# LouisBearing/BirdSoundClassif

Hardware: AMD Instinct MI355X
Metric: clips/sec (3 s @ 22.05 kHz) detect fwd (higher is better)
Workload: dtype f32; 1 GPU; BASELINE.json configs[1]: 1xMI355X inference, batch=64 synthetic 3 s clips (PCM16 @22.05 kHz resident in HBM) through the HIP STFT front end + detector forward + device post-processing, detections returned to the host; batch_per_gpu=64, distinct_clips=64, lanes=2

## Files before the change

### birdsoundclassif_amd/_lib.py

```python
import ctypes as C
import os
import subprocess

_HERE = os.path.dirname(os.path.abspath(__file__))
LIB_PATH = os.environ.get('NBM_LIB') or os.path.join(_HERE, 'libnbm_hip.so')
CSRC = os.path.join(_HERE, 'csrc')

_lib = None


class GemmDesc(C.Structure):
    _fields_ = [('x', C.c_void_p), ('w', C.c_void_p), ('y', C.c_void_p),
                ('scale', C.c_void_p), ('shift', C.c_void_p), ('residual', C.c_void_p),
                ('x_gs', C.c_int64), ('w_gs', C.c_int64), ('y_gs', C.c_int64), ('res_gs', C.c_int64),
                ('groups', C.c_int),
                ('B', C.c_int), ('H', C.c_int), ('W', C.c_int), ('Cin', C.c_int),
                ('N', C.c_int),
                ('kh', C.c_int), ('kw', C.c_int), ('stride', C.c_int), ('pad', C.c_int),
                ('Ho', C.c_int), ('Wo', C.c_int),
                ('x_ld', C.c_int), ('w_ld', C.c_int), ('y_ld', C.c_int), ('res_ld', C.c_int),
                ('alpha', C.c_float), ('act', C.c_int), ('shift_per_row', C.c_int),
                ('up', C.c_void_p), ('up_H', C.c_int), ('up_W', C.c_int),
                ('rows', C.c_void_p), ('rows_blocks', C.c_void_p),
                ('rows_mode', C.c_int), ('rows_count', C.c_int), ('rows_TH', C.c_int), ('rows_TW', C.c_int),
                ('mask', C.c_void_p), ('mask_ld', C.c_int), ('bits_out', C.c_void_p)]


class GconvDesc(C.Structure):
    _fields_ = [('x', C.c_void_p), ('w', C.c_void_p), ('y', C.c_void_p), ('scale', C.c_void_p), ('shift', C.c_void_p),
                ('B', C.c_int), ('H', C.c_int), ('W', C.c_int), ('groups', C.c_int), ('Cg', C.c_int),
                ('kh', C.c_int), ('kw', C.c_int), ('stride', C.c_int), ('pad', C.c_int), ('Ho', C.c_int), ('Wo', C.c_int),
                ('x_ld', C.c_int), ('y_ld', C.c_int), ('relu', C.c_int)]


class GconvBwdDesc(C.Structure):
    _fields_ = [('g', C.c_void_p), ('y', C.c_void_p), ('w', C.c_void_p), ('x', C.c_void_p), ('out', C.c_void_p),
                ('scale', C.c_void_p), ('workspace', C.c_void_p), ('workspace_bytes', C.c_longlong),
                ('B', C.c_int), ('H', C.c_int), ('W', C.c_int), ('groups', C.c_int), ('Cg', C.c_int),
                ('kh', C.c_int), ('kw', C.c_int), ('stride', C.c_int), ('pad', C.c_int), ('Ho', C.c_int), ('Wo', C.c_int),
                ('g_ld', C.c_int), ('y_ld', C.c_int), ('x_ld', C.c_int), ('out_ld', C.c_int),
                ('accumulate', C.c_int), ('splits', C.c_int)]


class RoiDesc(C.Structure):
    _fields_ = [('fmap', C.c_void_p * 5), ('fh', C.c_int * 5), ('fw', C.c_int * 5),
                ('n_levels', C.c_int), ('C', C.c_int),
                ('rois', C.c_void_p), ('n_roi', C.c_void_p), ('B', C.c_int), ('roi_cap', C.c_int),
                ('pe_f', C.c_void_p), ('pe_t', C.c_void_p), ('img_h', C.c_int), ('img_w', C.c_int),
                ('pool', C.c_void_p), ('pe', C.c_void_p), ('level', C.c_void_p)]


class AugmentParams(C.Structure):
    _fields_ = [('gain', C.c_float), ('coef', C.c_float), ('denom', C.c_float), ('neg_coef', C.c_float),
                ('neg_denom', C.c_float), ('flags', C.c_int32), ('hard_index', C.c_int32), ('pad', C.c_int32),
                ('noise_seed', C.c_uint64)]


class BwdDesc(C.Structure):
    _fields_ = [('g', C.c_void_p), ('w', C.c_void_p), ('x', C.c_void_p), ('out', C.c_void_p),
                ('a_scale', C.c_void_p), ('row_scale', C.c_void_p), ('residual', C.c_void_p), ('mask', C.c_void_p),
                ('g_gs', C.c_int64), ('w_gs', C.c_int64), ('x_gs', C.c_int64), ('out_gs', C.c_int64), ('res_gs', C.c_int64),
                ('groups', C.c_int),
                ('B', C.c_int), ('H', C.c_int), ('W', C.c_int), ('Cin', C.c_int), ('N', C.c_int),
                ('kh', C.c_int), ('kw', C.c_int), ('stride', C.c_int), ('pad', C.c_int), ('Ho', C.c_int), ('Wo', C.c_int),
                ('g_ld', C.c_int), ('w_ld', C.c_int), ('x_ld', C.c_int), ('out_ld', C.c_int), ('res_ld', C.c_int),
                ('mask_ld', C.c_int), ('alpha', C.c_float), ('bias_grad', C.c_void_p), ('residual2', C.c_void_p), ('res2_ld', C.c_int),
                ('mask_bits', C.c_void_p)]


class GemmPlan(C.Structure):
    _fields_ = [('name', C.c_char_p), ('rc', C.c_int), ('kernel', C.c_int), ('grid', C.c_int * 3), ('block', C.c_int),
                ('m_tiles', C.c_int), ('n_tiles', C.c_int), ('vec_epi', C.c_int), ('fast', C.c_int), ('slices', C.c_int),
                ('phased', C.c_int), ('ph_tiles', C.c_int * 4), ('splits', C.c_int), ('k_chunk', C.c_int),
                ('plain', C.c_int), ('b_generic', C.c_int), ('narrow_m', C.c_int), ('halves', C.c_int)]


_P, _I, _L, _F, _U64 = C.c_void_p, C.c_int, C.c_int64, C.c_float, C.c_uint64

SIGNATURES = {
    'nbm_graph_census': [_P, C.POINTER(C.c_longlong * 6)],
    'nbm_copy_rect': [_P, _P, _L, _L, _I, _L, _L, _I, _I, _P],
    'nbm_gemm_conv': [C.POINTER(GemmDesc), _P],
    'nbm_gconv3x3': [C.POINTER(GconvDesc), _P],
    'nbm_gconv3x3_dgrad': [C.POINTER(GconvBwdDesc), _P],
    'nbm_gconv3x3_wgrad': [C.POINTER(GconvBwdDesc), _P],
    'nbm_gconv3x3_wgrad_workspace': [C.POINTER(GconvBwdDesc), C.POINTER(C.c_longlong)],
    'nbm_pcm16_to_wave': [_P, _L, _I, _I, _I, _P, _L, _L, _P, _L, _I, _I, _P],
    'nbm_resample_to_wave': [_P, _L, _I, _L, _I, _I, _P, _I, _L, _L, _P, _L, _I, _I, _I, _P],
    'nbm_wav_decode': [_P, _L, _I, _I, _I, _I, _L, _P, _L, _P],
    'nbm_minmax_init': [_P, _I, _P],
    'nbm_stft_db': [_P, _L, _I, _I, _I, _I, _P, _I, _I, _I, _F, _P, _L, _I, _P, _P],
    'nbm_spec_windows': [_P, _L, _I, _I, _I, _I, _P, _P, _I, _I, _I, _P, _P],
    'nbm_spec_windows_table': [_P, _I, _I, _P, _I, _I, _P],
    'nbm_init_conv': [_P, _L, _P, _P, _I, _P, _P],
    'nbm_stem7x7': [_P, _I, _I, _I, _P, _P, _P, _P, _P, _P, _P],
    'nbm_stem7x7_wgrad': [_P, _P, _I, _I, _I, _P, _P, _P],
    'nbm_maxpool3x3s2': [_P, _I, _I, _I, _I, _P, _I, _I, _P, _P],
    'nbm_space_to_batch2': [_P, _I, _I, _I, _I, _P, _I, _P],
    'nbm_avgpool2x2': [_P, _I, _I, _I, _I, _P, _P],
    'nbm_avgpool2x2_bwd': [_P, _I, _I, _I, _I, _P, _P],
    'nbm_upsample_bilinear_add': [_P, _I, _I, _I, _I, _P, _P, _I, _I, _P],
    'nbm_softmax_rows': [_P, _L, _I, _L, _P],
    'nbm_dwconv3x3': [_P, _I, _I, _I, _I, _I, _I, _P, _P, _P, _L, _P, _I, _I, _P],
    'nbm_silu': [_P, _P, _L, _P],
    'nbm_layernorm': [_P, _L, _I, _P, _P, _F, _P, _P],
    'nbm_mha_small': [_P, _P, _P, _I, _I, _I, _P, _I, _I, _I, _I, _I, _L, _L, _P, _F, _P],
    'nbm_mha_segments': [_P, _P, _P, _I, _I, _I, _P, _I, _I, _I, _I, _I, _I, _P, _P, _I, _F, _P],
    'nbm_pair_softmax': [_P, _L, _I, _I, _P, _I, _P],
    'nbm_rpn_decode': [_P, _P, _P, _I, _I, _I, _I, _I, _I, _P, _P, _P, _P],
    'nbm_nan_images': [_P, _I, _L, _P, _P],
    'nbm_rpn_select': [_P, _P, _P, _I, _I, _I, _I, _I, _P, _P, _P, _P, _P],
    'nbm_nms_batched': [_P, _P, _P, _I, _I, _F, _I, _P, _P, _P, _P, _P, _P, _P],
    'nbm_rpn_select_big_workspace': [_I, _I, C.POINTER(C.c_int64)],
    'nbm_rpn_select_big': [_P, _P, _P, _I, _I, _I, _I, _I, _P, _L, _P, _P, _P, _P, _P],
    'nbm_nms_big_workspace': [_I, _I, C.POINTER(C.c_int64)],
    'nbm_nms_big': [_P, _P, _P, _I, _I, _F, _I, _P, _L, _P, _P, _P, _P, _P],
    'nbm_roi_pool': [C.POINTER(RoiDesc), _P],
    'nbm_rcnn_post': [_P, _P, _I, _I, _P, _P, _I, _I, _I, _F, _F, _I, _P, _P, _P],
    'nbm_merge_collect': [_P, _P, _I, _I, _I, _I, _I, _L, _P, _P, _P, _P, _P, _P],
    'nbm_merge_nms_workspace': [_I, C.POINTER(C.c_int64)],
    'nbm_merge_nms': [_P, _P, _I, _F, _P, _L, _P, _P, _P],
    'nbm_merge_gather': [_P, _P, _P, _P, _P, _I, _P, _P, _P],
    'nbm_conv_dgrad': [C.POINTER(BwdDesc), _P],
    'nbm_conv_wgrad': [C.POINTER(BwdDesc), _P],
    'nbm_gemm_plan': [_I, _P, C.POINTER(GemmPlan)],
    'nbm_relu_bwd': [_P, _P, _P, _L, _P],
    'nbm_silu_bwd': [_P, _P, _P, _L, _P],
    'nbm_axpby': [_P, _P, _P, _F, _F, _L, _L, _P],
    'nbm_colsum': [_P, _L, _I, _I, _P, _P],
    'nbm_leaky_relu_bwd': [_P, _P, _P, _F, _L, _P],
    'nbm_layernorm_bwd': [_P, _P, _P, _L, _I, _F, _P, _P, _P, _P],
    'nbm_mha_small_bwd': [_P, _P, _P, _P, _I, _I, _I, _I, _P, _P, _P, _I, _I, _I, _P, _I, _I, _I, _I, _L, _L, _P, _F, _P],
    'nbm_zero_roi_windows': [_P, _I, _I, _I, _P, _P, _I, _I, _I, _P],
    'nbm_zero_pattern': [_P, _I, _I, _I, _I, _I, _P],
    'nbm_zero_tiles': [_P, _I, _I, _I, _I, _P, _I, _P, _P],
    'nbm_tiles_gather': [_P, _I, _I, _I, _I, _P, _I, _P, _P, _P],
    'nbm_tiles_scatter_add': [_P, _I, _I, _I, _I, _P, _I, _P, _P, _P],
    'nbm_proposal_iou': [_P, _P, _P, _I, _I, _I, _P, _P, _P],
    'nbm_anchor_targets': [_P, _I, _P, _P, _I, _I, _F, _F, _P, _P, _P, _P],
    'nbm_maxpool3x3s2_bwd': [_P, _P, _P, _I, _I, _I, _I, _I, _I, _P, _P, _P],
    'nbm_upsample_bilinear_bwd': [_P, _I, _I, _I, _I, _P, _I, _I, _I, _P],
    'nbm_tiles_upsample_bilinear_bwd_add': [_P, _I, _I, _I, _I, _P, _I, _P, _P, _I, _I, _P],
    'nbm_png_unfilter_gray8': [_P, _L, _I, _I, _I, _P, _L, _P, _P],
    'nbm_image_half_std_u8': [_P, _L, _I, _L, _P, _P],
    'nbm_randn_fill': [_U64, _L, _P, _P],
    'nbm_augment_batch': [_P, _P, _P, _I, _I, _I, _P, _P, _P, _P, _P, _P, _P],
    'nbm_u8_to_unit': [_P, _L, _P, _P],
    'nbm_wino_input': [_P, _I, _I, _I, _I, _P, _I, _P],
# ... 78 lines not shown
```

### birdsoundclassif_amd/csrc/stem.hip

```cpp
#include "nbm_common.h"

namespace {

constexpr int SP = 264;
constexpr int KR = 8;
constexpr int KK = 7 * KR;
constexpr int OP = 68;
static_assert(7 * SP + KK * 64 <= 128 * OP, "operands must fit the output tile");

struct StemParams {
  const float* img; const float* weff; const float* wb; const float* wb_full; const float* scale; const float* shift;
  float* y;
  int B, H, W, Ho, Wo;
};

__global__ __launch_bounds__(256) void stem7x7_kernel(const StemParams p) {
  __shared__ __attribute__((aligned(16))) float smem[128 * OP];
  float* img_s = smem;
  float* w_s = smem + 7 * SP;
  __shared__ float cb_s[64 * 8];
  const int tid = threadIdx.x, lane = tid & 63, wave = tid >> 6;
  const int ox0 = blockIdx.x * 128, oy = blockIdx.y, b = blockIdx.z;

  const int ix0 = 2 * ox0 - 3;
  constexpr int NST = (7 * SP + 255) / 256;
  float stv[NST];
#pragma unroll
  for (int k = 0; k < NST; ++k) {
    const int i = min(tid + 256 * k, 7 * SP - 1);
    const int r = i / SP, c = i - r * SP;
    const int iy = min(max(2 * oy - 3 + r, 0), p.H - 1), ix = min(max(ix0 + c, 0), p.W - 1);
    stv[k] = p.img[((long long)b * p.H + iy) * p.W + ix];
  }
#pragma unroll
  for (int k = 0; k < NST; ++k) {
    const int i = tid + 256 * k;
    const int r = i / SP, c = i - r * SP;
    const int iy = 2 * oy - 3 + r, ix = ix0 + c;
    if (i < 7 * SP) img_s[i] = ((unsigned)iy < (unsigned)p.H && (unsigned)ix < (unsigned)p.W && c < 261) ? stv[k] : 0.f;
  }
  for (int i = tid; i < KK * 64 / 4; i += 256)
    reinterpret_cast<f32x4*>(w_s)[i] = reinterpret_cast<const f32x4*>(p.weff)[i];
  unsigned rmask = 0;
#pragma unroll
  for (int r = 0; r < 7; ++r)
    if ((unsigned)(2 * oy - 3 + r) < (unsigned)p.H) rmask |= 1u << r;
  const bool row_border = rmask != 0x7fu;
  const bool col_border = ox0 < 2 || 2 * (ox0 + 127) + 3 >= p.W;
  if (row_border || col_border)
    for (int i = tid; i < 64 * 7; i += 256) {
      const int n = i / 7, sx = i - n * 7;
      float a = 0.f;
      for (int r = 0; r < 7; ++r)
// ... 1 lines not shown
      cb_s[n * 8 + sx] = a;
    }
  __syncthreads();

  const int pl = lane & 31, slot = lane >> 5;
  const float* a_base = img_s + 2 * (wave * 32 + pl) + slot;
  const float* b_base = w_s + slot * 64 + pl;
  f32x16 acc0, acc1;
#pragma unroll
  for (int e = 0; e < 16; ++e) { acc0[e] = 0.f; acc1[e] = 0.f; }
#pragma unroll
  for (int j = 0; j < KK / 2; ++j) {
    constexpr int dummy = 0; (void)dummy;
    const int r = (2 * j) / KR, s0 = (2 * j) % KR;
    const float a = a_base[r * SP + s0];
    const float b0 = b_base[(2 * j) * 64], b1 = b_base[(2 * j) * 64 + 32];
    acc0 = __builtin_amdgcn_mfma_f32_32x32x2f32(a, b0, acc0, 0, 0, 0);
    acc1 = __builtin_amdgcn_mfma_f32_32x32x2f32(a, b1, acc1, 0, 0, 0);
  }

  __syncthreads();
#pragma unroll
  for (int t = 0; t < 2; ++t) {
    const int n = 32 * t + pl;
    const float sc = p.scale[n], sh = p.shift[n];
    float bfull = p.wb_full[n];
    if (row_border) {
      bfull = 0.f;
#pragma unroll
      for (int s = 0; s < 7; ++s) bfull += cb_s[n * 8 + s];
    }
    const f32x16& acc = t == 0 ? acc0 : acc1;
#pragma unroll
    for (int e = 0; e < 16; ++e) {
      const int px = wave * 32 + (e & 3) + 8 * (e >> 2) + 4 * slot;
      const int ox = ox0 + px;
      float bias = bfull;
      if (col_border && (ox < 2 || 2 * ox + 3 >= p.W)) {
        bias = 0.f;
#pragma unroll
        for (int s = 0; s < 7; ++s)
          if ((unsigned)(2 * ox - 3 + s) < (unsigned)p.W) bias += cb_s[n * 8 + s];
      }
      smem[px * OP + n] = fmaxf((acc[e] + bias) * sc + sh, 0.f);
    }
  }
  __syncthreads();
  float* yrow = p.y + (((long long)b * p.Ho + oy) * p.Wo + ox0) * 64;
#pragma unroll
  for (int it = 0; it < 8; ++it) {
    const int px = it * 16 + (tid >> 4), c4 = (tid & 15) * 4;
    if (ox0 + px < p.Wo)
      *reinterpret_cast<f32x4*>(yrow + px * 64 + c4) = *reinterpret_cast<const f32x4*>(smem + px * OP + c4);
  }
}

struct StemWgradParams {
  const float* img; const float* g; float* D;
  int B, H, W, Ho, Wo, n_strips, tiles_x;
};

__global__ __launch_bounds__(256) void stem_wgrad_kernel(const StemWgradParams p) {
  __shared__ __attribute__((aligned(16))) float img_s[7 * SP];
  __shared__ __attribute__((aligned(16))) float g_s[128 * 64];
  const int tid = threadIdx.x, lane = tid & 63, wave = tid >> 6;
  const int mt = wave >> 1, nt = wave & 1;
  const int pl = lane & 31, slot = lane >> 5;
  const int col = nt * 32 + pl;
  const int r = col >> 3, sx = col & 7;
  const bool tap = col < 56 && sx < 7;
  const float ones = col == 56 ? 1.f : 0.f;
  const float* b_base = img_s + (tap ? r * SP + sx : 0) + 2 * slot;
  const float* a_base = g_s + slot * 64 + mt * 32 + pl;
  f32x16 acc;
#pragma unroll
  for (int e = 0; e < 16; ++e) acc[e] = 0.f;
  for (int strip = blockIdx.x; strip < p.n_strips; strip += gridDim.x) {
    const int tx = strip % p.tiles_x, rowi = strip / p.tiles_x;
    const int oy = rowi % p.Ho, b = rowi / p.Ho;
    const int ox0 = tx * 128, ix0 = 2 * ox0 - 3;
    __syncthreads();
    constexpr int NST = (7 * SP + 255) / 256;
    float stv[NST];
#pragma unroll
    for (int k = 0; k < NST; ++k) {
      const int i = min(tid + 256 * k, 7 * SP - 1);
      const int rr = i / SP, c = i - rr * SP;
      const int iy = min(max(2 * oy - 3 + rr, 0), p.H - 1), ix = min(max(ix0 + c, 0), p.W - 1);
      stv[k] = p.img[((long long)b * p.H + iy) * p.W + ix];
    }
    const float* gsrc = p.g + (((long long)b * p.Ho + oy) * p.Wo + ox0) * 64;
    const int npx = min(128, p.Wo - ox0);
    f32x4 gv[8];
#pragma unroll
    for (int k = 0; k < 8; ++k) {
      const int i = tid + 256 * k;
      gv[k] = *reinterpret_cast<const f32x4*>(gsrc + (long long)(min(i >> 4, npx - 1) * 16 + (i & 15)) * 4);
    }
#pragma unroll
    for (int k = 0; k < NST; ++k) {
      const int i = tid + 256 * k;
      const int rr = i / SP, c = i - rr * SP;
      const int iy = 2 * oy - 3 + rr, ix = ix0 + c;
      if (i < 7 * SP) img_s[i] = ((unsigned)iy < (unsigned)p.H && (unsigned)ix < (unsigned)p.W && c < 261) ? stv[k] : 0.f;
    }
#pragma unroll
// ... 43 lines not shown
      const bool rin = (unsigned)(2 * oy - 3 + r) < (unsigned)H;
#pragma unroll
      for (int s2 = 0; s2 < 7; ++s2) {
        const bool cin = (unsigned)(2 * ox - 3 + s2) < (unsigned)W;
        acc[r * 7 + s2] += (rin && cin) ? 0.f : gv;
      }
    }
  }
#pragma unroll
  for (int e = 0; e < 49; ++e) red[sub][n][e] = acc[e];
  __syncthreads();
  for (int i = threadIdx.x; i < 64 * 49; i += 256) {
    const int nn = i / 49, e = i - nn * 49;
    const float v = red[0][nn][e] + red[1][nn][e] + red[2][nn][e] + red[3][nn][e];
    if (v != 0.f) atomicAdd(Cb + i, v);
  }
}

}

extern "C" int nbm_stem7x7_wgrad(const float* img, const float* g, int B, int H, int W, float* D, float* Cb, void* stream) {
  if (!img || !g || !D || !Cb || B <= 0 || H <= 0 || W <= 0) return NBM_EINVAL;
  if (!nbm_aligned16(g)) return NBM_EALIGN;
  StemWgradParams p{};
  p.img = img; p.g = g; p.D = D; p.B = B; p.H = H; p.W = W;
  p.Ho = (H + 6 - 7) / 2 + 1; p.Wo = (W + 6 - 7) / 2 + 1;
  p.tiles_x = (p.Wo + 127) / 128;
  const long long strips = (long long)B * p.Ho * p.tiles_x;
  if (strips > 0x7fffffffll) return NBM_EUNSUPPORTED;
  p.n_strips = (int)strips;
  hipStream_t st = (hipStream_t)stream;
  if (nbm_zero_async(D, sizeof(float) * 64 * 64, st) != hipSuccess || nbm_zero_async(Cb, sizeof(float) * 64 * 49, st) != hipSuccess)
    return (int)hipGetLastError();
  const int grid = (int)(strips < 1024 ? strips : 1024);
  hipLaunchKernelGGL(stem_wgrad_kernel, dim3(grid), dim3(256), 0, st, p);
  int top = p.Ho < 2 ? p.Ho : 2, bot0 = top, left = p.Wo < 2 ? p.Wo : 2, right0 = left;
  while (bot0 < p.Ho && 2 * bot0 + 3 < H) ++bot0;
  while (right0 < p.Wo && 2 * right0 + 3 < W) ++right0;
  hipLaunchKernelGGL(stem_vborder_kernel, dim3(8, B), dim3(256), 0, st, g, H, W, p.Ho, p.Wo, top, bot0, left, right0, Cb);
  return nbm_launch_status();
}

extern "C" int nbm_stem7x7(const float* img, int B, int H, int W, const float* weff, const float* wb, const float* wb_full,
                           const float* scale, const float* shift, float* y, void* stream) {
  if (!img || !weff || !wb || !wb_full || !scale || !shift || !y || B <= 0 || H <= 0 || W <= 0) return NBM_EINVAL;
  if (!nbm_aligned16(weff)) return NBM_EALIGN;
  StemParams p{};
  p.img = img; p.weff = weff; p.wb = wb; p.wb_full = wb_full; p.scale = scale; p.shift = shift; p.y = y;
  p.B = B; p.H = H; p.W = W; p.Ho = (H + 6 - 7) / 2 + 1; p.Wo = (W + 6 - 7) / 2 + 1;
  dim3 grid((p.Wo + 127) / 128, p.Ho, B);
  hipLaunchKernelGGL(stem7x7_kernel, grid, dim3(256), 0, (hipStream_t)stream, p);
  return nbm_launch_status();
}
```

### birdsoundclassif_amd/nets/backbone.py

```python
import torch
from torch import nn

from .. import ops
from . import _prep, functional as Fn
from .position_encoding import build_position_encoding

bcbk_channels = {'resnet': {'2': 64, '3': 256, '4': 512, '5': 1024, '6': 2048}}
_RESNET_LAYERS = {'resnet50': [3, 4, 6, 3], 'resnet101': [3, 4, 23, 3], 'resnet152': [3, 8, 36, 3]}
_RESNEXT = {'resnext50_32x4d': ([3, 4, 6, 3], 32, 4), 'resnext101_32x8d': ([3, 4, 23, 3], 32, 8),
            'resnext101_64x4d': ([3, 4, 23, 3], 64, 4)}


class FrozenBatchNorm2d(nn.Module):

    def __init__(self, n):
        super().__init__()
        self.register_buffer('weight', torch.ones(n))
        self.register_buffer('bias', torch.zeros(n))
        self.register_buffer('running_mean', torch.zeros(n))
        self.register_buffer('running_var', torch.ones(n))

    def _load_from_state_dict(self, state_dict, prefix, local_metadata, strict, missing_keys, unexpected_keys,
                              error_msgs):
        state_dict.pop(prefix + 'num_batches_tracked', None)
# ... 54 lines not shown
        self.bn3 = norm_layer(planes * 4)
        self.downsample = downsample
        self.stride, self.groups = stride, groups
        self.mask_input, self.mask_gy = False, True

    def forward(self, x):
        grad = torch.is_grad_enabled() and (x.requires_grad or any(p.requires_grad for p in self.parameters()))
        if grad and not self.training:
            raise NotImplementedError('a ResNeXt block in eval mode has no backward pass: call .train() on the model to train through it '
                                      '(FrozenBN makes the two modes compute the same), or train with --lr_backbone 0 (a frozen '
                                      'backbone), or run it under torch.no_grad()')
        s, b = self.bn1.affine()
        o = Fn.conv(x, self.conv1.weight, scale=s, shift=b, act=ops.ACT_RELU)
        s, b = self.bn2.affine()
        if grad:
            o = Fn.GConv3x3.apply(o, self.conv2.weight, s, b, self.groups, self.stride)
        else:
            o = ops.gconv3x3(o, _prep.gconv(self.conv2.weight, self.groups), self.groups, stride=self.stride, scale=s, shift=b, relu=True)
        if self.downsample is not None:
            s, b = self.downsample[1].affine()
            idt = Fn.conv(x, self.downsample[0].weight, scale=s, shift=b, stride=self.stride)
        else:
            idt = x
        s, b = self.bn3.affine()
        return Fn.conv(o, self.conv3.weight, scale=s, shift=b, residual=idt, act=ops.ACT_RELU)


class _ResNetBody(nn.Module):

    def __init__(self, layers, norm_layer, dilation=False, groups=1, base_width=64):
        super().__init__()
        self.conv1 = nn.Conv2d(3, 64, 7, stride=2, padding=3, bias=False)
        self.bn1 = norm_layer(64)
        self.dilation = bool(dilation)
        inplanes = 64
        for li, (planes, n, stride) in enumerate(zip((64, 128, 256, 512), layers, (1, 2, 2, 1 if dilation else 2)), start=1):
            blocks = []
            for bi in range(n):
                st = stride if bi == 0 else 1
                ds = None
                if bi == 0 and (st != 1 or inplanes != planes * 4):
                    ds = nn.Sequential(nn.Conv2d(inplanes, planes * 4, 1, stride=st, bias=False), norm_layer(planes * 4))
                blocks.append(_Bottleneck(inplanes, planes, st, ds, norm_layer) if groups == 1 else
                              _GroupedBottleneck(inplanes, planes, st, ds, norm_layer, groups, base_width))
                if dilation and li == 4 and bi > 0:
                    blocks[-1].conv2.dilation, blocks[-1].conv2.padding = (2, 2), (2, 2)
                blocks[-1].mask_input = not (li == 1 and bi == 0)
                blocks[-1].mask_gy = bi == n - 1
                inplanes = planes * 4
            setattr(self, f'layer{li}', nn.Sequential(*blocks))

    def forward(self, x, init_conv=None):
        s, b = self.bn1.affine()
        if init_conv is not None:
            x = Fn.Stem.apply(x, init_conv.weight, init_conv.bias, self.conv1.weight, s, b)
        else:
            x = Fn.conv(x, self.conv1.weight, scale=s, shift=b, kh=7, kw=7, stride=2, pad=3, act=ops.ACT_RELU)
        taps = [x]
        x = Fn.MaxPool.apply(x, True)
        for li in range(1, 5):
            for bi, blk in enumerate(getattr(self, f'layer{li}')):
                if self.dilation and li == 4 and bi == 1:
                    x = Fn.SpaceToBatch2.apply(x, False)
                x = blk(x)
            if self.dilation and li == 4 and len(self.layer4) > 1:
                x = Fn.SpaceToBatch2.apply(x, True)
            taps.append(x)
        return taps


class BackboneBase(nn.Module):

    def __init__(self, backbone, name, in_channels, train_backbone):
        super().__init__()
        for _, parameter in backbone.named_parameters():
            if not train_backbone:
                parameter.requires_grad_(False)
        self.body = backbone
        self.num_channels = list(bcbk_channels['resnet'].values())
        if in_channels != 3:
            self.init_conv = nn.Conv2d(in_channels, 3, 1)
        self.in_channels = in_channels
        self.strides = [2 ** (i + 1) for i in range(len(self.num_channels))]

    def forward(self, x):
        if hasattr(self, 'init_conv'):
            if self.in_channels != 1:
                raise NotImplementedError('init_conv is implemented for 1 input channel (reference default)')
            return self.body(x, self.init_conv)
        return self.body(x)


class Backbone(BackboneBase):

    def __init__(self, name, in_channels, train_backbone, dilation, norm_layer_name):
        if name not in _RESNET_LAYERS and name not in _RESNEXT:
            raise ValueError(f'not supported {name}: the accelerated path implements {sorted(_RESNET_LAYERS) + sorted(_RESNEXT)}')
        if norm_layer_name != 'frozen_batchnorm':
            raise NotImplementedError('only --norm_layer_backbone frozen_batchnorm (reference default) is implemented')
        layers, groups, base_width = _RESNEXT[name] if name in _RESNEXT else (_RESNET_LAYERS[name], 1, 64)
        super().__init__(_ResNetBody(layers, FrozenBatchNorm2d, dilation=dilation, groups=groups, base_width=base_width), name,
                         in_channels, train_backbone)
        if groups > 1 and not train_backbone and hasattr(self, 'init_conv'):
            self.init_conv.requires_grad_(False)


class Joiner(nn.Sequential):
    def __init__(self, backbone, position_embedding):
        super().__init__(backbone, position_embedding)

    def forward(self, x):
        return self[0](x), None
# ... 12 lines not shown
```

### birdsoundclassif_amd/nets/functional.py

```python
import os
import weakref

import torch
from torch.autograd import Function
from torch.autograd.function import once_differentiable

from .. import ops, ondemand
from . import _prep

ACT_NONE, ACT_RELU, ACT_LEAKY = ops.ACT_NONE, ops.ACT_RELU, ops.ACT_LEAKY


def _pad32_rows(g2d, n):
    n32 = (n + 31) // 32 * 32
    if n32 == n:
        return g2d
    out = torch.zeros((g2d.shape[0], n32), device=g2d.device, dtype=torch.float32)
    out[:, :n] = g2d
    return out


GRAD_SINK = {}


# ... 534 lines not shown
    @staticmethod
    def forward(ctx, x, weight, bias, eps):
        ctx.save_for_backward(x, weight)
        ctx.eps = eps
        return ops.layernorm(x, weight.detach(), bias.detach(), eps)

    @staticmethod
    @once_differentiable
    def backward(ctx, g):
        x, weight = ctx.saved_tensors
        gx, gw, gb = ops.layernorm_bwd(x, weight.detach(), g.contiguous(), ctx.eps)
        return gx, gw, gb, None


class MhaSmall(Function):

    @staticmethod
    def forward(ctx, q, k, v, S, N, nhead, seq_stride, batch_stride, n_valid):
        ctx.save_for_backward(q, k, v, n_valid)
        ctx.geom = (S, N, nhead, seq_stride, batch_stride)
        return ops.mha_small(q, k, v, S, N, nhead, seq_stride, batch_stride, n_valid)

    @staticmethod
    @once_differentiable
    def backward(ctx, go):
        q, k, v, n_valid = ctx.saved_tensors
        gq, gk, gv = ops.mha_small_bwd(q, k, v, go.contiguous(), *ctx.geom, n_valid)
        return gq, gk, gv, None, None, None, None, None, None


class Stem(Function):

    @staticmethod
    def forward(ctx, x, w_init, b_init, w1, scale, shift):
        y = ops.stem7x7(x, *_prep.stem_fold(w1, w_init, b_init), scale, shift)
        ctx.save_for_backward(x, w_init, b_init, w1, scale, y)
        return y

    @staticmethod
    @once_differentiable
    def backward(ctx, gy):
        x, w_init, b_init, w1, scale, y = ctx.saved_tensors
        g = gy.contiguous() if _premasked(y, gy) else ops.relu_bwd(gy.contiguous(), y)
        U, V = ops.stem7x7_wgrad(x, g)
        U, V = U * scale.view(64, 1, 1), V * scale.view(64, 1, 1)
        wi, bi = w_init.detach().view(3), b_init.detach().view(3)
        gw1 = wi.view(1, 3, 1, 1) * U[:, None] + bi.view(1, 3, 1, 1) * V[:, None]
        w1d = w1.detach()
        gwi = (w1d * U[:, None]).sum(dim=(0, 2, 3)).view_as(w_init)
        gbi = (w1d * V[:, None]).sum(dim=(0, 2, 3))
        return None, gwi, gbi, gw1, None, None


class MaxPool(Function):

    @staticmethod
    def forward(ctx, x, relu_input=False):
        y, idx = ops.maxpool3x3s2(x, with_index=True)
        ctx.hw = x.shape[1:3]
        ctx.x_ptr, ctx.take_x = x.data_ptr(), stash_accept(x, ctx.needs_input_grad[0])
        ctx.premask = bool(relu_input and ctx.take_x)
        ctx.save_for_backward(idx, x if ctx.premask else None)
        return y

    @staticmethod
    @once_differentiable
    def backward(ctx, gy):
        idx, x = ctx.saved_tensors
        other = _STASH.pop(ctx.x_ptr, None) if ctx.take_x else None
        premask = ctx.premask and other is not None
        gx = ops.maxpool3x3s2_bwd(idx, gy.contiguous(), *ctx.hw, residual=other, mask=x if premask else None)
        ondemand.zero_recycle(other)
        if premask:
            _PREMASKED[ctx.x_ptr] = (gx.data_ptr(), gx._version)
        return gx, None


class SpaceToBatch2(Function):

    @staticmethod
    def forward(ctx, x, inverse):
        ctx.inverse = bool(inverse)
        return ops.space_to_batch2(x, inverse=ctx.inverse)

    @staticmethod
    @once_differentiable
    def backward(ctx, gy):
        return ops.space_to_batch2(gy.contiguous(), inverse=not ctx.inverse), None


class AvgPool2x2(Function):

    @staticmethod
    def forward(ctx, x):
        return ops.avgpool2x2(x)

    @staticmethod
    @once_differentiable
    def backward(ctx, gy):
        return ops.avgpool2x2_bwd(gy.contiguous())


class UpsampleAdd(Function):
    @staticmethod
    def forward(ctx, src, add, Ho, Wo):
        ctx.hw = src.shape[1:3]
# ... 354 lines not shown
```

### birdsoundclassif_amd/ops.py

```python
import collections
import ctypes as C
import os
import math

import torch

from . import _lib
from ._lib import GconvBwdDesc, GconvDesc, GemmDesc, RoiDesc, check

ACT_NONE, ACT_RELU, ACT_SILU, ACT_LEAKY = 0, 1, 2, 3

PROFILE = None
FLOPS = None
FLOPS_DEFERRED = []


def flops_total():
    tot = FLOPS[0] + sum(float(c.item()) * f for c, f in FLOPS_DEFERRED)
    FLOPS_DEFERRED.clear()
    return tot


_PROFILE_LABEL = None
PROFILE_ONLY = None
# ... 444 lines not shown


def window_entry(db, minmax, last_cols, window, n_img):
    import numpy as np
    _chk(db, name='db'), _chk(last_cols, torch.int32, 'last_cols')
    if db.dim() != 2 or db.stride(1) != 1 or minmax.dtype != torch.int32 or minmax.numel() != 2 or not minmax.is_contiguous():
        raise ValueError('window_entry: db [n_bins, n_frames] with unit column stride, minmax int32 [2]')
    if not 0 <= window < n_img:
        raise ValueError('window_entry: window index outside the file')
    lo = lambda a, b: (int(a) & 0xffffffff) | (int(b) << 32)
    return np.array([db.data_ptr(), minmax.data_ptr(), last_cols.data_ptr(), lo(db.stride(0), db.shape[1]), lo(window, n_img)],
                    dtype=np.int64)


def spec_windows_table(table, n_bins, w_pix, hop_img, out=None):
    _chk(table, torch.int64, 'table')
    if table.dim() != 2 or table.shape[1] != WINDOW_ENTRY_WORDS:
        raise ValueError(f'window table of shape {tuple(table.shape)}: expected (B, {WINDOW_ENTRY_WORDS})')
    B = table.shape[0]
    img = out if out is not None else torch.empty((B, n_bins, w_pix), device=table.device, dtype=torch.float32)
    _chk(img, name='img')
    assert tuple(img.shape) == (B, n_bins, w_pix)
    check(lib().nbm_spec_windows_table(_ptr(table), B, n_bins, _ptr(img), w_pix, hop_img, _stream()), 'nbm_spec_windows_table')
    return img


def init_conv(x, w, b):
    _chk(x, name='x')
    C_ = w.numel()
    y = torch.empty(x.shape[:3] + (C_,), device=x.device, dtype=torch.float32)
    check(lib().nbm_init_conv(_ptr(x), x.numel(), _ptr(_chk(w.reshape(-1))), _ptr(_chk(b)), C_, _ptr(y), _stream()),
          'nbm_init_conv')
    return y


def stem7x7(img, weff, wb, wb_full, scale, shift):
    _chk(img, name='img')
    B, H, W = img.shape[:3]
    assert img.numel() == B * H * W and tuple(weff.shape) == (56, 64)
    y = torch.empty((B, (H - 1) // 2 + 1, (W - 1) // 2 + 1, 64), device=img.device, dtype=torch.float32)
    if FLOPS is not None:
        FLOPS[0] += 2.0 * y.numel() * 56
    if _prof_all():
        ev = (torch.cuda.Event(enable_timing=True), torch.cuda.Event(enable_timing=True))
        ev[0].record()
    check(lib().nbm_stem7x7(_ptr(img), B, H, W, _ptr(_chk(weff)), _ptr(_chk(wb)), _ptr(_chk(wb_full)), _ptr(_chk(scale)),
                            _ptr(_chk(shift)), _ptr(y), _stream()), 'nbm_stem7x7')
    if _prof_all():
        ev[1].record()
        PROFILE.append(((1, 64, 7, H, W, B, 1, 2, None), *ev))
    return y


def stem7x7_wgrad(img, g):
    _chk(img, name='img'), _chk(g, name='g')
    B, H, W = img.shape[:3]
    assert g.shape == (B, (H - 1) // 2 + 1, (W - 1) // 2 + 1, 64)
    D = torch.empty((64, 64), device=img.device, dtype=torch.float32)
    Cb = torch.empty((64, 49), device=img.device, dtype=torch.float32)
    check(lib().nbm_stem7x7_wgrad(_ptr(img), _ptr(g), B, H, W, _ptr(D), _ptr(Cb), _stream()), 'nbm_stem7x7_wgrad')
    U = D[:, :56].view(64, 7, 8)[:, :, :7]
    V = D[:, 56].view(64, 1, 1) - Cb.view(64, 7, 7)
    return U, V


def maxpool3x3s2(x, with_index=False):
    _chk(x, name='x')
    B, H, W, C_ = x.shape
    Ho, Wo = (H - 1) // 2 + 1, (W - 1) // 2 + 1
    y = torch.empty((B, Ho, Wo, C_), device=x.device, dtype=torch.float32)
    idx = torch.empty((B, Ho, Wo, C_), device=x.device, dtype=torch.uint8) if with_index else None
    check(lib().nbm_maxpool3x3s2(_ptr(x), B, H, W, C_, _ptr(y), Ho, Wo, _ptr(idx), _stream()), 'nbm_maxpool3x3s2')
    return (y, idx) if with_index else y


def space_to_batch2(x, inverse=False):
    _chk(x, name='x')
    if inverse:
        B4, h, w, C_ = x.shape
        assert B4 % 4 == 0
        B, H, W = B4 // 4, 2 * h, 2 * w
        y = torch.empty((B, H, W, C_), device=x.device, dtype=torch.float32)
    else:
        B, H, W, C_ = x.shape
        if (H | W) & 1:
            raise NotImplementedError('space_to_batch2 needs even map sizes (the dilated ResNet stage at 24 x 64)')
        y = torch.empty((4 * B, H // 2, W // 2, C_), device=x.device, dtype=torch.float32)
    check(lib().nbm_space_to_batch2(_ptr(x), B, H, W, C_, _ptr(y), int(bool(inverse)), _stream()), 'nbm_space_to_batch2')
    return y


def avgpool2x2(x):
    _chk(x, name='x')
    B, H, W, C_ = x.shape
    assert H % 2 == 0 and W % 2 == 0
    y = torch.empty((B, H // 2, W // 2, C_), device=x.device, dtype=torch.float32)
    check(lib().nbm_avgpool2x2(_ptr(x), B, H // 2, W // 2, C_, _ptr(y), _stream()), 'nbm_avgpool2x2')
    return y


def avgpool2x2_bwd(gy):
    _chk(gy, name='gy')
    B, Ho, Wo, C_ = gy.shape
    gx = torch.empty((B, 2 * Ho, 2 * Wo, C_), device=gy.device, dtype=torch.float32)
    check(lib().nbm_avgpool2x2_bwd(_ptr(gy), B, Ho, Wo, C_, _ptr(gx), _stream()), 'nbm_avgpool2x2_bwd')
    return gx
# ... 812 lines not shown
```

### include/nbm_hip.h

```cpp
#ifndef NBM_HIP_H
#define NBM_HIP_H

#include <stdint.h>

#ifdef __cplusplus
extern "C" {
#endif

#define NBM_OK 0
#define NBM_EINVAL (-1)
#define NBM_EALIGN (-2)
#define NBM_EUNSUPPORTED (-3)

#define NBM_ACT_NONE 0
#define NBM_ACT_RELU 1
#define NBM_ACT_SILU 2
#define NBM_ACT_LEAKY 3

const char* nbm_version(void);

int nbm_graph_census(void* graph, long long counts[6]);

typedef struct nbm_gemm_desc {
  const float* x;
// ... 95 lines not shown
                   int c_off , void* stream);
int nbm_cell_input_up(const float* x1, const float* bias, int B, int H, int W, int C, int Hc, int Wc, int stride, float* Vx, int ld,
                      int c_off, void* stream);
int nbm_cell_patches(const float* x, int B, int H, int W, int C, int stride, float* Vx, int ld, int c_off, void* stream);
int nbm_cell_patches_up(const float* x1, const float* bias, int B, int H, int W, int C, int Hc, int Wc, int stride, float* Vx, int ld,
                        int c_off, void* stream);
int nbm_cell_patches_up_cols(const float* x1, const float* bias, int B, int H, int W, int C, int Hc, int Wc, int stride, float* Vx,
                             void* stream);

int nbm_copy_rect(float* strided, float* packed, int64_t n_outer, int64_t outer_pitch, int n_rows, int64_t row_pitch, int64_t width,
                  int to_strided, int zero_strided, void* stream);
int nbm_cell_dgrad_output(const float* M, int B, int H, int W, int C, int stride, float* gx, int parity_class,
                          int ld , int c_off ,
                          float* bias_grad , void* stream);
int nbm_cell_output(const float* M, const float* bias, int B, int H, int W, int N, int stride, float* y, void* stream);


int nbm_pcm16_to_wave(const int16_t* pcm, int64_t pcm_ld, int batch, int n, int upsample,
                      const int32_t* hq, int64_t first, int64_t count, float* out, int64_t out_ld, int lead,
                      int pad_mode, void* stream);

int nbm_resample_to_wave(const float* x, int64_t x_ld, int batch, int64_t n, int L, int M, const double* taps, int T,
                         int64_t first, int64_t count, float* out, int64_t out_ld, int lead, int pad_mode, int quant16,
                         void* stream);

#define NBM_WAV_MAX_CHANNELS 8
int nbm_wav_decode(const void* raw, int64_t raw_pitch, int batch, int tag, int bits, int channels, int64_t n, float* out,
                   int64_t out_pitch, void* stream);

int nbm_minmax_init(uint32_t* minmax, int batch, void* stream);
int nbm_stft_db(const float* wave, int64_t wave_ld, int batch, int n_frames, int hop, int n_fft,
                const double* basis, int basis_bin_tiles, int basis_ksteps, int n_bins, float floor_amp,
                float* db, int64_t db_bs, int db_ld, uint32_t* minmax, void* stream);

int nbm_spec_windows(const float* db, int64_t db_bs, int db_ld, int batch, int n_bins, int n_frames,
                     const uint32_t* minmax, float* img, int n_img, int w_pix, int hop_img,
                     const int32_t* last_cols, void* stream);

typedef struct nbm_window_entry {
  const float* db;
  const uint32_t* minmax;
  const int32_t* last_cols;
  int32_t db_ld, n_frames, window, n_img;
} nbm_window_entry;

int nbm_spec_windows_table(const nbm_window_entry* table, int batch, int n_bins, float* img, int w_pix, int hop_img,
                           void* stream);


int nbm_init_conv(const float* x, int64_t n_pix, const float* w, const float* b, int C, float* y, void* stream);

int nbm_stem7x7(const float* img, int B, int H, int W, const float* weff, const float* wb, const float* wb_full,
                const float* scale, const float* shift, float* y, void* stream);

int nbm_stem7x7_wgrad(const float* img, const float* g, int B, int H, int W, float* D, float* Cb, void* stream);

int nbm_maxpool3x3s2(const float* x, int B, int H, int W, int C, float* y, int Ho, int Wo, uint8_t* idx, void* stream);
int nbm_space_to_batch2(const float* x, int B, int H, int W, int C, float* y, int inverse, void* stream);
int nbm_avgpool2x2(const float* x, int B, int Ho, int Wo, int C, float* y, void* stream);
int nbm_avgpool2x2_bwd(const float* gy, int B, int Ho, int Wo, int C, float* gx, void* stream);

int nbm_upsample_bilinear_add(const float* src, int B, int Hi, int Wi, int C, const float* add,
                              float* y, int Ho, int Wo, void* stream);

int nbm_softmax_rows(float* x, int64_t rows, int cols, int64_t ld, void* stream);

int nbm_dwconv3x3(const float* x, int B, int H, int W, int Cin, int mult, int stride,
                  const float* w , const float* bias, const float* film, int64_t film_ld,
                  float* y, int Ho, int Wo, void* stream);

int nbm_silu(const float* x, float* y, int64_t n, void* stream);

int nbm_layernorm(const float* x, int64_t rows, int E, const float* w, const float* b, float eps, float* y, void* stream);

int nbm_mha_small(const float* q, const float* k, const float* v, int q_ld, int k_ld, int v_ld, float* out, int out_ld,
                  int S, int N, int nhead, int hd, int64_t seq_stride, int64_t batch_stride, const int32_t* n_valid,
                  float scale, void* stream);

#define NBM_MHA_ACROSS_ROIS 0
#define NBM_MHA_ACROSS_IMAGES 1
int nbm_mha_segments(const float* q, const float* k, const float* v, int q_ld, int k_ld, int v_ld, float* out, int out_ld,
                     int B, int R, int nhead, int hd, int mode, const int32_t* segments, const int32_t* n_roi, int max_count,
                     float scale, void* stream);

int nbm_pair_softmax(const float* x, int64_t n_pix, int n_anchor, int x_ld, float* y, int y_ld, void* stream);


int nbm_rpn_decode(const float* cls, const float* reg, const float* anchors , int B, int KA,
                   int n_anchor , int img_w, int img_h, int min_size, float* boxes,
                   uint32_t* keys, int* keep_count, void* stream);

int nbm_nan_images(const float* img, int B, int64_t n, int* keep_count, void* stream);


int nbm_rpn_select(const float* boxes, const uint32_t* keys, const int* keep_count, int B, int KA,
                   int top_n, int fail_below, int cap, float* sel_boxes, float* sel_scores, int* n_sel,
                   const int* seg, void* stream);

int nbm_nms_batched(const float* boxes, const float* scores, const int* n_in, int B, int cap, float thresh,
                    int post_n, uint64_t* mask_ws, int* keep_ws, float* rois, float* roi_scores, int* n_out,
                    const int* seg, void* stream);

int nbm_rpn_select_big_workspace(int B, int cap, int64_t* bytes);
int nbm_rpn_select_big(const float* boxes, const uint32_t* keys, const int* keep_count, int B, int KA, int top_n,
                       int fail_below, int cap, void* ws, int64_t ws_bytes, float* sel_boxes, float* sel_scores,
                       int* n_sel, const int* seg, void* stream);
// ... 155 lines not shown
```

Before: 1095 clips/s.

## Fuse stem 7x7 conv with 3x3 stride-2 maxpool in one banded kernel

Adds a stem kernel that computes the 7x7 stride-2 conv+BN+ReLU over row bands and overlapping 128-pixel column strips, and applies the 3x3/2 max-pool from the shared-memory tile before writing. The full-resolution stem output is still written because it is a tap, but the separate maxpool kernel, its re-read of that output and one launch go away. In exchange, rows and columns on band and strip edges are recomputed. The kernel also uses more shared memory for the band image, which may lower occupancy. Inference uses the fused path by default when no gradients are needed.

```diff
diff --git a/birdsoundclassif_amd/_lib.py b/birdsoundclassif_amd/_lib.py
--- a/birdsoundclassif_amd/_lib.py
+++ b/birdsoundclassif_amd/_lib.py
@@ -73,6 +73,16 @@
                 ('m_tiles', C.c_int), ('n_tiles', C.c_int), ('vec_epi', C.c_int), ('fast', C.c_int), ('slices', C.c_int),
                 ('phased', C.c_int), ('ph_tiles', C.c_int * 4), ('splits', C.c_int), ('k_chunk', C.c_int),
                 ('plain', C.c_int), ('b_generic', C.c_int), ('narrow_m', C.c_int), ('halves', C.c_int)]
+
+
+class StemPoolPlan(C.Structure):
+    _fields_ = [('rc', C.c_int), ('Ho', C.c_int), ('Wo', C.c_int), ('Hp', C.c_int), ('Wp', C.c_int),
+                ('strips', C.c_int), ('bands', C.c_int),
+                ('col_first', C.c_int), ('col_step', C.c_int), ('cols', C.c_int), ('col_keep_lo', C.c_int), ('col_keep', C.c_int),
+                ('pcols', C.c_int),
+                ('row_first', C.c_int), ('row_step', C.c_int), ('rows', C.c_int), ('row_keep_lo', C.c_int), ('row_keep', C.c_int),
+                ('prows', C.c_int),
+                ('grid', C.c_int * 3), ('block', C.c_int)]
 
 
 _P, _I, _L, _F, _U64 = C.c_void_p, C.c_int, C.c_int64, C.c_float, C.c_uint64
@@ -94,6 +104,8 @@
     'nbm_spec_windows_table': [_P, _I, _I, _P, _I, _I, _P],
     'nbm_init_conv': [_P, _L, _P, _P, _I, _P, _P],
     'nbm_stem7x7': [_P, _I, _I, _I, _P, _P, _P, _P, _P, _P, _P],
+    'nbm_stem7x7_pool': [_P, _I, _I, _I, _P, _P, _P, _P, _P, _P, _P, _P],
+    'nbm_stem_pool_plan': [_I, _I, _I, C.POINTER(StemPoolPlan)],
     'nbm_stem7x7_wgrad': [_P, _P, _I, _I, _I, _P, _P, _P],
     'nbm_maxpool3x3s2': [_P, _I, _I, _I, _I, _P, _I, _I, _P, _P],
     'nbm_space_to_batch2': [_P, _I, _I, _I, _I, _P, _I, _P],
diff --git a/birdsoundclassif_amd/csrc/stem.hip b/birdsoundclassif_amd/csrc/stem.hip
--- a/birdsoundclassif_amd/csrc/stem.hip
+++ b/birdsoundclassif_amd/csrc/stem.hip
@@ -1,4 +1,5 @@
 #include "nbm_common.h"
+#include "stem_pool_plan.h"
 
 namespace {
 
@@ -106,6 +107,161 @@
     const int px = it * 16 + (tid >> 4), c4 = (tid & 15) * 4;
     if (ox0 + px < p.Wo)
       *reinterpret_cast<f32x4*>(yrow + px * 64 + c4) = *reinterpret_cast<const f32x4*>(smem + px * OP + c4);
+  }
+}
+
+struct StemPoolParams {
+  const float* img; const float* weff; const float* wb; const float* wb_full; const float* scale; const float* shift;
+  float* y; float* yp;
+  int B, H, W, Ho, Wo, Hp, Wp, R;
+};
+
+constexpr int BAND_IN = 4 * nbm_stem_pool::BAND_POOLED + 7;
+constexpr int PSTEP = nbm_stem_pool::STRIP_STEP;
+constexpr int PCOLS = nbm_stem_pool::STRIP_POOLED;
+static_assert(nbm_stem_pool::STRIP_COLS == 128 && 2 * 127 + 7 < SP, "the strip is the 128-pixel MFMA tile of stem7x7_kernel");
+
+__device__ __forceinline__ f32x4 max4(f32x4 a, f32x4 b) {
+  f32x4 m = {fmaxf(a[0], b[0]), fmaxf(a[1], b[1]), fmaxf(a[2], b[2]), fmaxf(a[3], b[3])};
+  return m;
+}
+
+__global__ __launch_bounds__(256) void stem7x7_pool_kernel(const StemPoolParams p) {
+  __shared__ __attribute__((aligned(16))) float tile[128 * OP];
+  __shared__ __attribute__((aligned(16))) float img_s[BAND_IN * SP];
+  __shared__ float cb_s[64 * 8];
+  const int tid = threadIdx.x, lane = tid & 63, wave = tid >> 6;
+  const int pl = lane & 31, slot = lane >> 5;
+  const int b = blockIdx.z;
+  const int ox0 = (int)blockIdx.x * PSTEP - 1, ix0 = 2 * ox0 - 3;
+  const int p0 = (int)blockIdx.y * p.R, p1 = min(p0 + p.R, p.Hp);
+  const int oy_first = max(2 * p0 - 1, 0), oy_last = min(2 * p1 - 1, p.Ho - 1);
+  const float* img_b = p.img + (long long)b * p.H * p.W;
+  const bool wave_live = ox0 + wave * 32 < p.Wo;
+  const bool col_border = ox0 < 2 || 2 * (ox0 + 127) + 3 >= p.W;
+
+  float bw0[KK / 2], bw1[KK / 2];
+#pragma unroll
+  for (int j = 0; j < KK / 2; ++j) {
+    bw0[j] = p.weff[(2 * j + slot) * 64 + pl];
+    bw1[j] = p.weff[(2 * j + slot) * 64 + 32 + pl];
+  }
+  float sc[2], sh[2], wbf[2];
+#pragma unroll
+  for (int t = 0; t < 2; ++t) { sc[t] = p.scale[32 * t + pl]; sh[t] = p.shift[32 * t + pl]; wbf[t] = p.wb_full[32 * t + pl]; }
+
+  const int iy0 = 2 * oy_first - 3, n_in = 2 * (oy_last - oy_first) + 7;
+  for (int base = 0; base < n_in * SP; base += 8 * 256) {
+    float stv[8];
+#pragma unroll
+    for (int k = 0; k < 8; ++k) {
+      const int i = min(base + tid + 256 * k, n_in * SP - 1);
+      const int r = i / SP, c = i - r * SP;
+      const int iy = min(max(iy0 + r, 0), p.H - 1), ix = min(max(ix0 + c, 0), p.W - 1);
+      stv[k] = img_b[(long long)iy * p.W + ix];
+    }
+#pragma unroll
+    for (int k = 0; k < 8; ++k) {
+      const int i = base + tid + 256 * k;
+      const int r = i / SP, c = i - r * SP;
+      const int iy = iy0 + r, ix = ix0 + c;
+      if (i < n_in * SP) img_s[i] = ((unsigned)iy < (unsigned)p.H && (unsigned)ix < (unsigned)p.W && c < 261) ? stv[k] : 0.f;
+    }
+  }
+
+  const float* a_base = img_s + 2 * (wave * 32 + pl) + slot;
+  const int c4 = (tid & 15) * 4, jr = tid >> 4;
+  const f32x4 ninf = {-INFINITY, -INFINITY, -INFINITY, -INFINITY};
+  f32x4 vm[4] = {ninf, ninf, ninf, ninf};
+  unsigned cb_rmask = ~0u;
+
+  for (int oy = oy_first; oy <= oy_last; ++oy) {
+    unsigned rmask = 0;
+#pragma unroll
+    for (int r = 0; r < 7; ++r)
+      if ((unsigned)(2 * oy - 3 + r) < (unsigned)p.H) rmask |= 1u << r;
+    const bool row_border = rmask != 0x7fu;
+    if ((row_border || col_border) && rmask != cb_rmask) {
+      for (int i = tid; i < 64 * 7; i += 256) {
+        const int n = i / 7, sx = i - n * 7;
+        float a = 0.f;
+        for (int r = 0; r < 7; ++r)
+          if ((rmask >> r) & 1u) a += p.wb[n * 49 + r * 7 + sx];
+        cb_s[n * 8 + sx] = a;
+      }
+      cb_rmask = rmask;
+    }
+    __syncthreads();
+
+    if (wave_live) {
+      const float* a_row = a_base + 2 * (oy - oy_first) * SP;
+      f32x16 acc0, acc1;
+#pragma unroll
+      for (int e = 0; e < 16; ++e) { acc0[e] = 0.f; acc1[e] = 0.f; }
+#pragma unroll
+      for (int j = 0; j < KK / 2; ++j) {
+        const int r = (2 * j) / KR, s0 = (2 * j) % KR;
+        const float a = a_row[r * SP + s0];
+        acc0 = __builtin_amdgcn_mfma_f32_32x32x2f32(a, bw0[j], acc0, 0, 0, 0);
+        acc1 = __builtin_amdgcn_mfma_f32_32x32x2f32(a, bw1[j], acc1, 0, 0, 0);
+      }
+      int Wv = p.W, oxv = ox0;
+      asm volatile("" : "+s"(Wv), "+s"(oxv));
+#pragma unroll
+      for (int t = 0; t < 2; ++t) {
+        const int n = 32 * t + pl;
+        float bfull = wbf[t];
+        if (row_border) {
+          bfull = 0.f;
+#pragma unroll
+          for (int s = 0; s < 7; ++s) bfull += cb_s[n * 8 + s];
+        }
+        const f32x16& acc = t == 0 ? acc0 : acc1;
+#pragma unroll
+        for (int e = 0; e < 16; ++e) {
+          const int px = wave * 32 + (e & 3) + 8 * (e >> 2) + 4 * slot;
+          const int ox = oxv + px;
+          float bias = bfull;
+          if (col_border && (ox < 2 || 2 * ox + 3 >= Wv)) {
+            bias = 0.f;
+#pragma unroll
+            for (int s = 0; s < 7; ++s)
+              if ((unsigned)(2 * ox - 3 + s) < (unsigned)Wv) bias += cb_s[n * 8 + s];
+          }
+          tile[px * OP + n] = fmaxf((acc[e] + bias) * sc[t] + sh[t], 0.f);
+        }
+      }
+    }
+    __syncthreads();
+
+    const bool keep_row = oy >= 2 * p0;
+    const bool odd = oy & 1;
+    const int pr = oy >> 1;
+    const bool emit = (odd || oy == p.Ho - 1) && pr >= p0;
+    float* yrow = p.y + ((long long)b * p.Ho + oy) * p.Wo * 64;
+    float* prow = p.yp + ((long long)b * p.Hp + pr) * p.Wp * 64;
+#pragma unroll
+    for (int it = 0; it < 4; ++it) {
+      const int jj = it * 16 + jr;
+      const int col1 = ox0 + 2 * jj + 1;
+      if (jj < PCOLS && col1 < p.Wo) {
+        const float* tp = tile + (2 * jj) * OP + c4;
+        const f32x4 v0 = *reinterpret_cast<const f32x4*>(tp);
+        const f32x4 v1 = *reinterpret_cast<const f32x4*>(tp + OP);
+        const f32x4 v2 = *reinterpret_cast<const f32x4*>(tp + 2 * OP);
+        const bool right = col1 + 1 < p.Wo;
+        if (keep_row) {
+          *reinterpret_cast<f32x4*>(yrow + (unsigned)(col1 * 64 + c4)) = v1;
+          if (right) *reinterpret_cast<f32x4*>(yrow + (unsigned)(col1 * 64 + 64 + c4)) = v2;
+        }
+        f32x4 h = v1;
+        if (col1 > 0) h = max4(h, v0);
+        if (right) h = max4(h, v2);
+        vm[it] = max4(vm[it], h);
+        if (emit) *reinterpret_cast<f32x4*>(prow + (unsigned)(((int)blockIdx.x * PCOLS + jj) * 64 + c4)) = vm[it];
+        if (odd) vm[it] = h;
+      }
+    }
   }
 }
 
@@ -255,3 +411,23 @@
   hipLaunchKernelGGL(stem7x7_kernel, grid, dim3(256), 0, (hipStream_t)stream, p);
   return nbm_launch_status();
 }
+
+extern "C" int nbm_stem7x7_pool(const float* img, int B, int H, int W, const float* weff, const float* wb, const float* wb_full,
+                                const float* scale, const float* shift, float* y, float* yp, void* stream) {
+  if (!img || !weff || !wb || !wb_full || !scale || !shift || !y || !yp) return NBM_EINVAL;
+  const nbm_stem_pool::StemPoolPlan pl = nbm_stem_pool::plan(B, H, W);
+  if (pl.rc != NBM_OK) return pl.rc;
+  if (pl.prows > nbm_stem_pool::BAND_POOLED) return NBM_EUNSUPPORTED;
+  if (!nbm_aligned16(y) || !nbm_aligned16(yp)) return NBM_EALIGN;
+  StemPoolParams p{};
+  p.img = img; p.weff = weff; p.wb = wb; p.wb_full = wb_full; p.scale = scale; p.shift = shift; p.y = y; p.yp = yp;
+  p.B = B; p.H = H; p.W = W; p.Ho = pl.Ho; p.Wo = pl.Wo; p.Hp = pl.Hp; p.Wp = pl.Wp; p.R = pl.prows;
+  hipLaunchKernelGGL(stem7x7_pool_kernel, dim3(pl.grid[0], pl.grid[1], pl.grid[2]), dim3(pl.block), 0, (hipStream_t)stream, p);
+  return nbm_launch_status();
+}
+
+extern "C" int nbm_stem_pool_plan(int B, int H, int W, nbm_stem_pool_plan_t* out) {
+  if (!out) return NBM_EINVAL;
+  *out = nbm_stem_pool::plan(B, H, W);
+  return out->rc;
+}
diff --git a/birdsoundclassif_amd/csrc/stem_pool_plan.h b/birdsoundclassif_amd/csrc/stem_pool_plan.h
--- /dev/null
+++ b/birdsoundclassif_amd/csrc/stem_pool_plan.h
@@ -0,0 +1,34 @@
+#pragma once
+#include "nbm_hip.h"
+
+namespace nbm_stem_pool {
+
+constexpr int STRIP_COLS = 128;
+constexpr int STRIP_POOLED = (STRIP_COLS - 2) / 2;
+constexpr int STRIP_STEP = 2 * STRIP_POOLED;
+constexpr int BAND_POOLED = 6;
+constexpr int GRID_YZ_MAX = 65535;
+constexpr int ROW_PIXELS_MAX = 1 << 24;
+
+using StemPoolPlan = nbm_stem_pool_plan_t;
+
+inline StemPoolPlan plan(int B, int H, int W) {
+  StemPoolPlan pl{};
+  if (B <= 0 || H <= 0 || W <= 0) { pl.rc = NBM_EINVAL; return pl; }
+  pl.Ho = (H - 1) / 2 + 1; pl.Wo = (W - 1) / 2 + 1;
+  pl.Hp = (pl.Ho - 1) / 2 + 1; pl.Wp = (pl.Wo - 1) / 2 + 1;
+  pl.strips = (pl.Wp + STRIP_POOLED - 1) / STRIP_POOLED;
+  pl.bands = (pl.Hp + BAND_POOLED - 1) / BAND_POOLED;
+  const int R = (pl.Hp + pl.bands - 1) / pl.bands;
+  pl.col_first = -1; pl.col_step = STRIP_STEP; pl.cols = STRIP_COLS;
+  pl.col_keep_lo = 1; pl.col_keep = STRIP_STEP; pl.pcols = STRIP_POOLED;
+  pl.row_first = -1; pl.row_step = 2 * R; pl.rows = 2 * R + 1;
+  pl.row_keep_lo = 1; pl.row_keep = 2 * R; pl.prows = R;
+  if (pl.bands > GRID_YZ_MAX || B > GRID_YZ_MAX || pl.Wo > ROW_PIXELS_MAX) { pl.rc = NBM_EUNSUPPORTED; return pl; }
+  pl.grid[0] = pl.strips; pl.grid[1] = pl.bands; pl.grid[2] = B;
+  pl.block = 256;
+  pl.rc = NBM_OK;
+  return pl;
+}
+
+}
diff --git a/birdsoundclassif_amd/nets/backbone.py b/birdsoundclassif_amd/nets/backbone.py
--- a/birdsoundclassif_amd/nets/backbone.py
+++ b/birdsoundclassif_amd/nets/backbone.py
@@ -130,12 +130,16 @@
 
     def forward(self, x, init_conv=None):
         s, b = self.bn1.affine()
-        if init_conv is not None:
-            x = Fn.Stem.apply(x, init_conv.weight, init_conv.bias, self.conv1.weight, s, b)
-        else:
-            x = Fn.conv(x, self.conv1.weight, scale=s, shift=b, kh=7, kw=7, stride=2, pad=3, act=ops.ACT_RELU)
-        taps = [x]
-        x = Fn.MaxPool.apply(x, True)
+        if init_conv is not None and Fn.stem_pool_fused(x, init_conv.weight, init_conv.bias, self.conv1.weight):
+            t, x = Fn.stem_pool(x, init_conv.weight, init_conv.bias, self.conv1.weight, s, b)
+            taps = [t]
+        else:
+            if init_conv is not None:
+                x = Fn.Stem.apply(x, init_conv.weight, init_conv.bias, self.conv1.weight, s, b)
+            else:
+                x = Fn.conv(x, self.conv1.weight, scale=s, shift=b, kh=7, kw=7, stride=2, pad=3, act=ops.ACT_RELU)
+            taps = [x]
+            x = Fn.MaxPool.apply(x, True)
         for li in range(1, 5):
             for bi, blk in enumerate(getattr(self, f'layer{li}')):
                 if self.dilation and li == 4 and bi == 1:
diff --git a/birdsoundclassif_amd/nets/functional.py b/birdsoundclassif_amd/nets/functional.py
--- a/birdsoundclassif_amd/nets/functional.py
+++ b/birdsoundclassif_amd/nets/functional.py
@@ -610,6 +610,16 @@
         return None, gwi, gbi, gw1, None, None
 
 
+def stem_pool_fused(x, *params):
+    if os.environ.get('NBM_STEM_POOL', '1')[:1] == '0':
+        return False
+    return not (torch.is_grad_enabled() and (x.requires_grad or any(q.requires_grad for q in params)))
+
+
+def stem_pool(x, w_init, b_init, w1, scale, shift):
+    return ops.stem7x7_pool(x, *_prep.stem_fold(w1, w_init, b_init), scale, shift)
+
+
 class MaxPool(Function):
 
     @staticmethod
diff --git a/birdsoundclassif_amd/ops.py b/birdsoundclassif_amd/ops.py
--- a/birdsoundclassif_amd/ops.py
+++ b/birdsoundclassif_amd/ops.py
@@ -520,6 +520,36 @@
     return y
 
 
+def stem7x7_pool(img, weff, wb, wb_full, scale, shift):
+    _chk(img, name='img')
+    B, H, W = img.shape[:3]
+    assert img.numel() == B * H * W and tuple(weff.shape) == (56, 64)
+    Ho, Wo = (H - 1) // 2 + 1, (W - 1) // 2 + 1
+    y = torch.empty((B, Ho, Wo, 64), device=img.device, dtype=torch.float32)
+    yp = torch.empty((B, (Ho - 1) // 2 + 1, (Wo - 1) // 2 + 1, 64), device=img.device, dtype=torch.float32)
+    if FLOPS is not None:
+        FLOPS[0] += 2.0 * y.numel() * 56
+    if _prof_all():
+        ev = (torch.cuda.Event(enable_timing=True), torch.cuda.Event(enable_timing=True))
+        ev[0].record()
+    check(lib().nbm_stem7x7_pool(_ptr(img), B, H, W, _ptr(_chk(weff)), _ptr(_chk(wb)), _ptr(_chk(wb_full)), _ptr(_chk(scale)),
+                                 _ptr(_chk(shift)), _ptr(y), _ptr(yp), _stream()), 'nbm_stem7x7_pool')
+    if _prof_all():
+        ev[1].record()
+        PROFILE.append(((1, 64, 7, H, W, B, 1, 2, ('stem-pool', yp.shape[1], yp.shape[2])), *ev))
+    return y, yp
+
+
+StemPoolPlan = collections.namedtuple('StemPoolPlan', 'rc Ho Wo Hp Wp strips bands col_first col_step cols col_keep_lo col_keep pcols '
+                                      'row_first row_step rows row_keep_lo row_keep prows grid block')
+
+
+def stem_pool_plan(B, H, W):
+    p = _lib.StemPoolPlan()
+    lib().nbm_stem_pool_plan(int(B), int(H), int(W), C.byref(p))
+    return StemPoolPlan(*(tuple(p.grid) if f == 'grid' else getattr(p, f) for f in StemPoolPlan._fields))
+
+
 def stem7x7_wgrad(img, g):
     _chk(img, name='img'), _chk(g, name='g')
     B, H, W = img.shape[:3]
diff --git a/include/nbm_hip.h b/include/nbm_hip.h
--- a/include/nbm_hip.h
+++ b/include/nbm_hip.h
@@ -171,6 +171,18 @@
 
 int nbm_stem7x7(const float* img, int B, int H, int W, const float* weff, const float* wb, const float* wb_full,
                 const float* scale, const float* shift, float* y, void* stream);
+
+int nbm_stem7x7_pool(const float* img, int B, int H, int W, const float* weff, const float* wb, const float* wb_full,
+                     const float* scale, const float* shift, float* y, float* yp, void* stream);
+typedef struct nbm_stem_pool_plan_t {
+  int rc;
+  int Ho, Wo, Hp, Wp;
+  int strips, bands;
+  int col_first, col_step, cols, col_keep_lo, col_keep, pcols;
+  int row_first, row_step, rows, row_keep_lo, row_keep, prows;
+  int grid[3], block;
+} nbm_stem_pool_plan_t;
+int nbm_stem_pool_plan(int B, int H, int W, nbm_stem_pool_plan_t* out);
 
 int nbm_stem7x7_wgrad(const float* img, const float* g, int B, int H, int W, float* D, float* Cb, void* stream);
 
```

After: 1101 clips/s, median of 3. No clear change (+0.5%).
